# marbl/parsnp

Hardware: AMD Instinct MI355X
Metric: genomes/sec (MUM+LCB end-to-end) (higher is better)
Workload: dtype int32

## Files before the change

parsnp_amd/csrc/engine/engine_core.h:

```cpp
#pragma once
#include <algorithm>
#include <atomic>
#include <chrono>
#include <cstdint>
#include <cstdio>
#include <cstdlib>
#include <cstring>
#include <memory>
#include <mutex>
#include <new>
#include <string>
#include <thread>
#include <vector>

#include "kernels.h"
#include "store_kernels.h"
#include "dense_kernels.h"
#include "index_kernels.h"
#include "snp_kernels.h"
#include "nj_kernels.h"

namespace pm {

struct HostPool {
// ... 177 lines not shown
    static constexpr size_t kCtrLost = kCtrBase + 7;
    static constexpr size_t kCtrWords = kCtrBase + 8;
    static_assert(kCtrErr < kCtrGrouped && kCtrGrouped < kCtrWide && kCtrWide + kCtrWideWords <= kCtrOverflow && kCtrOverflow < kCtrLost && kCtrLost < kCtrWords,
                  "the words of the counter block are distinct and inside it");

private:
    struct CallHint { int64_t units = 0, ncand = 0, nok = 0; };
    struct StoreCounts { int64_t ms_count, rg_count, layout_rows, rg_pkey_init; };
    StoreCounts store_mark() const { return StoreCounts{ms_count, rg_count, layout_rows, rg_pkey_init}; }
    void store_rewind(const StoreCounts& m) { ms_count = m.ms_count; rg_count = m.rg_count; layout_rows = m.layout_rows; rg_pkey_init = m.rg_pkey_init; }
    void store_reset() { store_rewind(StoreCounts{0, 0, -1, 0}); }

    struct SearchCall {
        const int64_t nreg; const int64_t* const starts; const int64_t* const lens; const int32_t* const minsize; BatchResult* const out;
        const bool want_events, mumi; const GapBatch* const gb;
        bool from_store = false;
        int nq = 0, no_small = 0, lbits = 0;
        size_t nrow = 0, regz = 0, bytes_R = 0, bytes_pre = 0;
        int64_t npairs = 0, npos = 0, tsize = 0, fwords = 0, tsize_clear = 0, fwords_clear = 0, nbk = 0, npos_bucketed = 0, nchunks = 0, centries = 0, nwv = 0;
        RegionInfo* R = nullptr; int64_t *posbase = nullptr, *cbase = nullptr, *stage = nullptr;
        std::vector<int64_t> bbase;
        uint32_t* d_err = nullptr;
        int64_t nflag = 0; uint64_t ovf_cap = 0; bool index_counts_read = false;
        CallHint none; CallHint* hint = nullptr;
        int64_t nunits = 0; bool units_known = false;
        size_t ev_guess = 0, slice_cap = 0, queue_cap = 0, grp_cap = 0;
        uint64_t nev = 0, nrest = 0, ngrp = 0, worst_slice = 0;
        uint32_t errbits = 0, sticky = 0;
        bool first_form = false, wide_form = false, grouping = false, by_buckets = false, coarse_by_buckets = false, sharded = false;
        uint64_t *skey = nullptr, *sval = nullptr;
        const int64_t* ncand_p = nullptr; bool anchor_guess = false;
        bool exact = false, anchor_call = false;
        int64_t ncand_i = 0, nok = 0; uint64_t ncand = 0; size_t nokz = 0; const int64_t* nok_p = nullptr;
        std::vector<uint64_t> counts, qcounts; int64_t nunits_live = 0;
        int32_t verdict = 0;
        std::vector<int32_t> reg_h; int64_t counts_h[2] = {0, 0};
    };
    static constexpr int kNext = 1, kRepeat = 2;

    int run_once(int64_t nreg, const int64_t* starts, const int64_t* lens, const int32_t* minsize, BatchResult* out, bool want_events,
                 bool mumi, const GapBatch* gb = nullptr) {
        SearchCall c{nreg, starts, lens, minsize, out, want_events, mumi, gb};
        int rc = plan_call(c);
        if (rc != kNext) return rc;
        upload_and_clear(c);
        if ((rc = build_index(c)) != kNext) return rc;
        if ((rc = count_units(c)) != kNext) return rc;
        if ((rc = search_events(c)) != kNext) return rc;
        order_events(c);
        if (mumi) return mumi_tail(c);
        if ((rc = master_ep(c)) != kNext) return rc;
        return candidate_tail(c);
    }

    int plan_call(SearchCall& c) {
        const int64_t nreg = c.nreg; const int64_t* const starts = c.starts; const int64_t* const lens = c.lens; const int32_t* const minsize = c.minsize;
        BatchResult* const out = c.out; const GapBatch* const gb = c.gb;
        timing.clear();
        const int nq = c.nq = ngen - 1;
        out->nregions = nreg; out->nq = nq; out->total = 0;
        out->off.assign((size_t)nreg + 1, 0);
        out->release();
        out->pool = pool;
        if (nreg == 0) return 0;
        if (nq < 1) { error = "need at least one query genome"; return -2; }
        const int no_small = c.no_small = c.mumi ? 1 : 0;
// ... 511 lines not shown
            if (coll.allgather(coll.ctx, send.data(), (int64_t)(sizeof(GenomeAtK) * send.size()), recv.data())) { error = "all-gather of candidate states failed"; return -4; }
            for (int r = 0; r < coll.world; r++) {
                int a, b; shard_range(ngen, r, coll.world, &a, &b);
                const GenomeAtK* src = recv.data() + (size_t)r * send.size();
                for (size_t k = 0; k < cz; k++)
                    for (int x = 0; x < b - a; x++) all[k * nqz + (size_t)(a - 1 + x)] = src[k * (size_t)widest + (size_t)x];
            }
            be.h2d(d_at.p, all.data(), sizeof(GenomeAtK) * all.size());
        }
        be.mark("fold");
        return 0;
    }

    int tail_attempt(SearchCall& c, const bool exact) {
        const int64_t nreg = c.nreg, nwv = c.nwv; const int nq = c.nq, lbits = c.lbits; const GapBatch* const gb = c.gb; BatchResult* const out = c.out;
        const bool from_store = c.from_store, sharded = c.sharded; CallHint& hint = *c.hint;
        uint64_t* const skey = c.skey; uint64_t* const sval = c.sval; const int64_t* const ncand_p = c.ncand_p;
        const int32_t& verdict = c.verdict;
        int64_t &ncand_i = c.ncand_i, &nok = c.nok; int64_t (&counts_h)[2] = c.counts_h; std::vector<int32_t>& reg_h = c.reg_h;
        c.exact = exact;
        ncand_i = 0;
        if (exact) be.d2h(&ncand_i, ncand_p, 8);
        if (verdict < 0) { budget_exceeded = true; error = "per-thread work budget exceeded on some rank (degenerate repeat structure in a region)"; return -5; }
        if (exact) {
            last_candidates = ncand_i;
            if (ncand_i == 0) { hint.ncand = 1; hint.nok = 0; if (resident && from_store) out->store_base = ms_count; be.mark(nullptr); collect_timing(); return 0; }
        }
        const uint64_t ncand = c.ncand = exact ? (uint64_t)ncand_i : (uint64_t)(hint.ncand + hint.ncand / 8 + 256);
        ensure(d_cand, (size_t)ncand);
        be.launch("cand_write", nwv * 64, CandWrite{d_R.p, nreg, d_posbase.p, d_wmask.p, d_woff.p, d_cand.p, ncand});
        const uint64_t* scand = d_cand.p;

        be.mark("fold");
        ensure(d_ok, (size_t)ncand); ensure(d_ok_k, (size_t)ncand); ensure(d_ok_lon, (size_t)ncand);
        ensure(d_osp, (size_t)ncand * (size_t)nq); ensure(d_ofwd, (size_t)ncand * (size_t)nq);
        const GenomeAtK* at = nullptr;
        if (sharded) {
            if (int rc = exchange_states(c)) return rc;
            at = d_at.p;
        }
        be.launch_wave("fold_candidates", xcd_grid((int64_t)ncand),
                       FoldCandidates{d_R.p, scand, ngen, at, skey, sval, d_lo.p, d_state.p, d_rep.p, lbits, d_cbase.p, d_coarse.p,
                                      d_ok_k.p, d_ok_lon.p, d_osp.p, d_ofwd.p, d_ok.p, (int64_t)ncand, ncand_p});

        be.mark("compact");
        ensure(d_okcnt, (size_t)ncand + 1); ensure(d_okpos, (size_t)ncand + 1);
        be.launch("ok_count", (int64_t)ncand + 1, OkCount{d_ok.p, ncand_p, d_okcnt.p, (int64_t)ncand});
        be.exclusive_scan(d_okcnt.p, d_okpos.p, (size_t)ncand + 1);
        const int64_t* nok_p = c.nok_p = d_okpos.p + ncand;
        nok = 0;
        if (exact) be.d2h(&nok, nok_p, 8);
        const size_t nokz = c.nokz = exact ? (size_t)nok : (size_t)ncand;
        ensure(d_creg, std::max<size_t>(nokz, 1)); ensure(d_ck, std::max<size_t>(nokz, 1)); ensure(d_clon, std::max<size_t>(nokz, 1));
        reg_h.assign(nokz, 0);
        out->release();
        out->kb = pool->take(4 * nokz); out->lonb = pool->take(4 * nokz);
        out->rows = want_rows; out->dirty_known = false; out->table_id = 0; out->store_base = -1;
        const StoreCounts before = store_mark();
        c.anchor_call = false;
        if (!want_rows) compact_sp(c); else compact_rows(c);
        be.d2h_async(reg_h.data(), d_creg.p, 4 * nokz);
        be.d2h_async(out->kb.p, d_ck.p, 4 * nokz);
        counts_h[0] = ncand_i; counts_h[1] = nok;
        if (!exact) { be.d2h_async(&counts_h[0], ncand_p, 8); be.d2h_async(&counts_h[1], nok_p, 8); }
        flush_downloads();
        be.mark(nullptr);
        be.sync();
        const bool anchor_call = c.anchor_call;
        if (!exact) {
            ncand_i = counts_h[0]; nok = counts_h[1];
            const bool fits = (uint64_t)ncand_i <= ncand && anchor_call == (nreg == 1 && !gb && nok >= dirty_min);
            if (!fits) {
                store_rewind(before);
                tail_repeats++;
                be.mark("candidates");
                return kRepeat;
            }
            last_candidates = ncand_i;
            if (out->store_base >= 0) ms_count = out->store_base + nok;
        }
        hint.ncand = std::max<int64_t>(ncand_i, 1); hint.nok = nok;
        last_accepted = nok;
        if (anchor_call) { anchor_table_rows = nok; anchor_table_id = out->table_id; }
        for (int64_t w = 0; w < nok; w++) out->off[(size_t)reg_h[(size_t)w] + 1]++;
        for (int64_t r = 0; r < nreg; r++) out->off[(size_t)r + 1] += out->off[(size_t)r];
        out->total = out->off[(size_t)nreg];
        if (out->table_id && out->store_base == 0) anchor_flags_h.assign(out->flags(), out->flags() + nok);
        return kNext;
    }

    void compact_sp(SearchCall& c) {
        const int nq = c.nq; const uint64_t ncand = c.ncand; const size_t nokz = c.nokz, nqz2 = (size_t)nq; BatchResult* const out = c.out;
        const uint64_t* const scand = d_cand.p; const int64_t* const ncand_p = c.ncand_p;
        ensure(d_csp, std::max<size_t>(nokz * nqz2, 1)); ensure(d_cfwd, std::max<size_t>(nokz * nqz2, 1));
        be.launch("compact_sp", (int64_t)ncand * nq,
                  CompactSp{scand, d_ok.p, d_okpos.p, nq, d_ok_k.p, d_ok_lon.p, d_osp.p, d_ofwd.p, d_creg.p, d_ck.p, d_clon.p, d_csp.p, d_cfwd.p, ncand_p});
        be.mark("download");
        group_downloads();
        out->spb = pool->take(4 * nokz * nqz2); out->fwdb = pool->take(nokz * nqz2);
        be.d2h_async(out->spb.p, d_csp.p, 4 * nokz * nqz2);
        be.d2h_async(out->fwdb.p, d_cfwd.p, nokz * nqz2);
        be.d2h_async(out->lonb.p, d_clon.p, 4 * nokz);
    }

    void compact_rows(SearchCall& c) {
        const int64_t nreg = c.nreg; const GapBatch* const gb = c.gb; const bool from_store = c.from_store, exact = c.exact, anchor_guess = c.anchor_guess;
        const int64_t nok = c.nok; const uint64_t ncand = c.ncand; const size_t nokz = c.nokz, ngz = (size_t)ngen; BatchResult* const out = c.out;
        const uint64_t* const scand = d_cand.p; const int64_t* const ncand_p = c.ncand_p; const int64_t* const nok_p = c.nok_p;
        bool& anchor_call = c.anchor_call;
        anchor_call = nreg == 1 && !gb && (exact ? nok >= dirty_min : anchor_guess);
        const bool keep_rows = resident && (anchor_call || from_store);
        const bool to_store = anchor_call || keep_rows;
        int32_t* p_start; uint8_t* p_strand; int32_t* p_lon; uint32_t* p_flags;
        if (to_store) {
            if (anchor_call) store_reset();
            const size_t base = (size_t)ms_count, upto = base + nokz;
            ensure_keep(d_anchor_start, std::max<size_t>(upto * ngz, 1), base * ngz); ensure_keep(d_ms_strand, std::max<size_t>(upto * ngz, 1), base * ngz);
            ensure_keep(d_anchor_lon, std::max<size_t>(upto, 1), base); ensure_keep(d_anchor_flags, std::max<size_t>(upto, 1), base);
            ensure_keep(d_ms_shift, std::max<size_t>(upto, 1), base); ensure_keep(d_ms_len, std::max<size_t>(upto, 1), base); ensure_keep(d_ms_state, std::max<size_t>(upto, 1), base);
            p_start = d_anchor_start.p + base * ngz; p_strand = d_ms_strand.p + base * ngz; p_lon = d_anchor_lon.p + base; p_flags = d_anchor_flags.p + base;
            out->store_base = (int64_t)base;
            ms_count = (int64_t)upto;
        } else {
            ensure(d_csp, std::max<size_t>(nokz * ngz, 1)); ensure(d_cfwd, std::max<size_t>(nokz * ngz, 1)); ensure(d_cflags, std::max<size_t>(nokz, 1));
            p_start = d_csp.p; p_strand = d_cfwd.p; p_lon = d_clon.p; p_flags = d_cflags.p;
        }
        const bool long_list = nreg == 1 && (exact ? nok >= dirty_min : anchor_guess);
        if (long_list) ensure(d_dirty, nokz);
        {
            const ClearJob jobs[] = {{p_flags, 4 * nokz, 0}, {long_list ? d_dirty.p : nullptr, long_list ? 4 * nokz : 0, 0},
                                     {to_store ? d_ms_shift.p + (ms_count - (int64_t)nokz) : nullptr, to_store ? 4 * nokz : 0, 0},
                                     {to_store ? d_ms_state.p + (ms_count - (int64_t)nokz) : nullptr, to_store ? nokz : 0, 0}};
            be.clear_many(jobs, 4);
        }
        be.launch("compact_candidates", (int64_t)ncand * ngen,
                  CompactCandidates{scand, d_ok.p, d_okpos.p, ngen, d_ok_k.p, d_ok_lon.p, d_osp.p, d_ofwd.p, d_starts.p, d_lens.p, d_glen,
                                    d_creg.p, d_ck.p, p_lon, p_start, p_strand, p_flags, ncand_p});
        if (long_list) {
            const int64_t nblocks = ((int64_t)nokz + kDirtyBlock - 1) / kDirtyBlock, groups = (ngen + 63) / 64;
            ensure(d_bmax, (size_t)nblocks * ngz); ensure(d_bmin, (size_t)nblocks * ngz);
            be.launch_wave("dirty_extent", nblocks * groups, DirtyExtent{p_start, p_lon, p_flags, nok_p, ngen, d_bmax.p, d_bmin.p});
            be.launch_wave("dirty_prefix", groups, DirtyPrefix{nblocks, ngen, d_bmax.p, d_bmin.p});
            be.launch_wave("dirty_mark", nblocks * groups, DirtyMark{p_start, p_lon, nok_p, ngen, d_bmax.p, d_bmin.p, p_flags, d_dirty.p});
            be.launch("dirty_merge", (int64_t)nokz, DirtyMerge{d_dirty.p, p_flags, nok_p});
            out->dirty_known = true;
        }
        if (to_store) {
            be.d2d(d_ms_len.p + (ms_count - (int64_t)nokz), p_lon, 4 * nokz);
            if (anchor_call) out->table_id = ++table_counter;
        }
        be.mark("download");
        group_downloads();
        out->flagsb = pool->take(4 * nokz);
        be.d2h_async(out->flagsb.p, p_flags, 4 * nokz);
        if (!keep_rows) {
            out->startb = pool->take(4 * nokz * ngz); out->strandb = pool->take(nokz * ngz);
            be.d2h_async(out->startb.p, p_start, 4 * nokz * ngz);
            be.d2h_async(out->strandb.p, p_strand, nokz * ngz);
        }
        be.d2h_async(out->lonb.p, p_lon, 4 * nokz);
    }

public:

    bool resident = false;
    int64_t ms_count = 0;
    int64_t rg_count = 0;
    std::vector<RegInfo> rg_info_h;
    std::vector<uint32_t> anchor_flags_h;
    static constexpr int kAgain = -6;

    void reset_call_counts() {
        last_positions = last_candidates = last_accepted = last_grouped = last_grouped_wide = last_wide_regions = 0; last_handed_back = -1;
        last_index_bucketed = last_index_overflow = 0; last_index_lost = -1; last_alg[0] = last_alg[1] = last_alg[2] = 0;
    }
    void begin_store_call() { timing.clear(); last_events = last_rest = 0; reset_call_counts(); }
    Store store_view() { return Store{d_anchor_start.p, d_ms_strand.p, d_anchor_lon.p, d_anchor_flags.p, d_ms_shift.p, d_ms_len.p, d_ms_state.p, ngen}; }
    Layout layout_view(uint64_t* image, bool coherent = true) { return Layout{image, d_lay_off.p, d_lay_bits.p, coherent ? 1 : 0}; }
    size_t layout_geometry() {
        const size_t ngz = (size_t)ngen;
        if (lay_words == 0) {
// ... 785 lines not shown
            be.launch("dense_rerank", n, DenseRerank{d_dval2.p, d_dhead.p, d_dfirst.p, d_drank[k + 1].p});
            L.lv[k + 1] = d_drank[k + 1].p;
            be.d2h(&groups, d_dfirst.p + n, 8);
            if (groups == n) break;
        }
        if (groups != n) { error = "suffix-array sort did not converge"; return -5; }
        dense_rounds = k + 1;
        L.top = k;
        be.launch("dense_lcp", n, DenseLcp{L, d_dval2.p, d_dstart.p, nflag, d_dlcp.p});
        be.launch("dense_rep", n, DenseRep{d_R.p, d_dlist.p, d_dval2.p, d_dstart.p, nflag, d_dlcp.p, d_rep.p});
        return 0;
    }
    bool dense_mode = false;
    std::vector<uint8_t> dense_h;
    void collect_timing_more() { for (const PhaseTime& t : be.collect()) timing.push_back(t); }

    int allgather_host(const void* send, int64_t bytes, void* recv) {
        if (!coll.device) return coll.allgather(coll.ctx, send, bytes, recv);
        ensure(d_hsend, (size_t)bytes); ensure(d_hrecv, (size_t)bytes * (size_t)coll.world);
        be.h2d(d_hsend.p, send, (size_t)bytes);
        if (be.allgather_dev(d_hsend.p, bytes, d_hrecv.p)) return 1;
        be.d2h(recv, d_hrecv.p, (size_t)bytes * (size_t)coll.world);
        return 0;
    }

    std::vector<uint64_t> ev_key_h, ev_val_h;
    std::vector<int32_t> rep_h;
    int ev_lbits = 0;
    int64_t work_budget = 1 << 22;
    int64_t dirty_min = 4096;
    int64_t flagged_div = 8;
    int64_t tangled_max = 1 << 17;
    bool fast_tail = true;
    int64_t tail_repeats = 0;
    bool tangle_rounds = true;
    bool group_small = true;
    bool group_wide = false;
    int64_t last_grouped = 0;
    int64_t last_grouped_wide = 0, last_handed_back = -1, last_wide_regions = 0;
    bool force_atomic_marks = false;
    int filter_factor = 8;
    int slot_factor = 2;
    bool bucket_sort = true;
    bool index_build = true;
    int64_t index_bucket_min = 1 << 24;
    bool index_verify = false;
    int64_t index_overflow_cap = 0;
    int64_t last_index_bucketed = 0, last_index_overflow = 0, last_index_lost = -1;
    bool master_seg = true;
    bool force_gate = false;
    int64_t chain_window = 4096;
    int64_t chain_passed[2] = {-1, -1};
    bool force_chain_tie = false;
    bool force_unsure = false;
    bool order_debug = false;
    int64_t outside_writes = 0;
    int64_t exact_cluster_tests = 0;
    int64_t deferred_regions = 0;
    bool clusters_out_of_order = false;
    int64_t hint_shrink = 1;
    bool phase_timing = true;
    bool tune(const std::string& key, int64_t value) {
        if (key == "flagged_div" && value >= 1) { flagged_div = value; return true; }
        if (key == "tangled_max" && value >= 0) { tangled_max = value; return true; }
        if (key == "tangle_rounds") { tangle_rounds = value != 0; return true; }
        if (key == "fast_tail") { fast_tail = value != 0; return true; }
        if (key == "atomic_marks") { force_atomic_marks = value != 0; return true; }
        if (key == "master_seg") { master_seg = value != 0; return true; }
        if (key == "bucket_sort") { bucket_sort = value != 0; return true; }
        if (key == "index_build") { index_build = value != 0; return true; }
        if (key == "index_bucket_min" && value >= 1) { index_bucket_min = value; return true; }
        if (key == "index_verify") { index_verify = value != 0; return true; }
        if (key == "index_overflow_cap" && value >= 0) { index_overflow_cap = value; return true; }
        if (key == "filter_factor") { filter_factor = value < 1 ? 1 : (int)value; return true; }
        if (key == "slot_factor") { slot_factor = value < 1 ? 1 : (int)value; return true; }
        if (key == "stage_gate") { force_gate = value != 0; return true; }
        if (key == "chain_window" && value >= 1 && value <= kChainWindowMax) { chain_window = value; return true; }
        if (key == "chain_tie") { force_chain_tie = value != 0; return true; }
        if (key == "cluster_unsure") { force_unsure = value != 0; return true; }
        if (key == "order_debug") { order_debug = value != 0; return true; }
        if (key == "timing") { phase_timing = value != 0; be.timing_on = phase_timing; return true; }
        if (key == "group_small") { group_small = value != 0; return true; }
        if (key == "group_wide") { group_wide = value != 0; return true; }
        if (key == "work_budget" && value > 0) { work_budget = value; return true; }
        if (key == "dense_all") { dense_all = value != 0; return true; }
        if (key == "dirty_min" && value >= 0) { dirty_min = value; return true; }
        if (key == "hint_shrink" && value >= 1) { hint_shrink = value; return true; }
        if (key == "copy_kernel") { return tune_copy_kernel(be, value != 0, 0); }
        return false;
    }

    void release() {
        if (chain_event) { be.event_wait(chain_event); be.event_release(chain_event); chain_event = nullptr; }
        for (BufBase* b : all_bufs) { if (b->raw) be.free(b->raw); b->raw = nullptr; b->cap = 0; }
        if (chain_host) be.pinned_free(chain_host);
        chain_host = nullptr; chain_host_cap = 0; chain_pending = false;
        if (blk) be.free(blk);
        if (d_goff) be.free(d_goff);
        if (d_glen) be.free(d_glen);
// ... 23 lines not shown
        if (n <= b.cap && b.p) return;
        if (std::find(all_bufs.begin(), all_bufs.end(), (BufBase*)&b) == all_bufs.end()) all_bufs.push_back(&b);
        const size_t want = n + n / 2 + 16;
        void* raw = be.alloc(want * sizeof(T));
        if (!raw) throw DeviceOutOfMemory{want * sizeof(T)};
        if (b.p && keep) { be.d2d(raw, b.p, keep * sizeof(T)); be.sync(); }
        if (b.raw) be.free(b.raw);
        b.raw = raw; b.p = (T*)raw; b.cap = want;
    }
    void collect_timing() { timing = be.collect(); }
    template <class T> static auto group_on(T& b, int) -> decltype(b.d2h_group(), void()) { b.d2h_group(); }
    template <class T> static void group_on(T&, long) {}
    template <class T> static auto flush_on(T& b, int) -> decltype(b.d2h_flush(), void()) { b.d2h_flush(); }
    template <class T> static void flush_on(T&, long) {}
    template <class T> static auto tune_copy_kernel(T& b, bool on, int) -> decltype(b.group_copies = on, true) { b.group_copies = on; return true; }
    template <class T> static bool tune_copy_kernel(T&, bool, long) { return true; }
    template <class T> static auto sort_keys_on(T& b, uint64_t* ki, uint64_t* ko, size_t n, int lo, int hi, int) -> decltype(b.sort_keys(ki, ko, n, lo, hi), true) { b.sort_keys(ki, ko, n, lo, hi); return true; }
    template <class T> static bool sort_keys_on(T&, uint64_t*, uint64_t*, size_t, int, int, long) { return false; }
    void group_downloads() { group_on(be, 0); }
    void flush_downloads() { flush_on(be, 0); }

    SeqBlock* blk = nullptr; int64_t* d_goff = nullptr; int64_t* d_glen = nullptr;
    Packed P{};
    size_t ev_cap_hint = 0, rest_cap_hint[2] = {0, 0}, grp_cap_hint = 0;
    std::vector<CallHint> call_hints;
    int64_t call_ordinal = 0;
    Buf<uint8_t> d_gflag; Buf<int64_t> d_glo;
    Buf<int64_t> d_bkbase, d_bkbegin, d_ovf; Buf<uint64_t> d_ikey, d_ikey2, d_ikey3, d_ikey4;
    Buf<RegionInfo> d_R; Buf<int64_t> d_starts, d_lens, d_posbase;
    Buf<uint64_t> d_slots; Buf<uint32_t> d_filter, d_repeated; Buf<int32_t> d_next, d_rep, d_run, d_epm;
    Buf<int64_t> d_ucount, d_uoff; Buf<UnitRec> d_units;
    Buf<uint64_t> d_counter, d_evkey, d_evval, d_evkey2, d_evval2, d_evkey3, d_evval3; Buf<int64_t> d_sliceoff;
    Buf<int64_t> d_lo, d_cov; Buf<EventAtK> d_state; Buf<PairState> d_wsummary, d_wcarry; Buf<int32_t> d_emax;
    Buf<uint64_t> d_cand; Buf<GenomeAtK> d_at; Buf<uint8_t> d_ok; Buf<int32_t> d_ok_k, d_ok_lon, d_osp; Buf<uint8_t> d_ofwd;
    Buf<uint64_t> d_wmask; Buf<int64_t> d_wcount, d_woff;
    Buf<int64_t> d_bcount, d_bbegin, d_pbase;
    Buf<int64_t> d_okcnt, d_okpos, d_cbase; Buf<int32_t> d_coarse; Buf<int32_t> d_creg, d_ck, d_clon, d_csp; Buf<uint8_t> d_cfwd;
    Buf<uint32_t> d_cflags, d_dirty; Buf<int32_t> d_bmax, d_bmin;
    Buf<GenomeAtK> d_xsend, d_xrecv; Buf<uint8_t> d_hsend, d_hrecv;
    Buf<RestItem> d_rest; Buf<uint64_t> d_qcount;
    Buf<uint8_t> d_dense; Buf<int32_t> d_dfi, d_dlist, d_dlcp; Buf<int64_t> d_dstart, d_dhead, d_dfirst;
    Buf<uint64_t> d_dkey, d_dkey2, d_dval, d_dval2; Buf<uint32_t> d_drank[kDenseMaxLevels];
    Buf<int32_t> d_anchor_start, d_anchor_lon; Buf<uint32_t> d_anchor_flags;
    int64_t table_counter = 0;
    Buf<uint64_t> d_image;
    Buf<int64_t> d_un_blk, d_un_cnt, d_un_scan, d_un_tot; Buf<int32_t> d_un_out;
    Buf<double> d_nj_D, d_nj_R, d_nj_q; Buf<uint8_t> d_nj_active; Buf<int32_t> d_nj_j, d_nj_dist; Buf<NjJoinRec> d_nj_joins; Buf<NjLastRec> d_nj_last;
    Buf<uint64_t> d_snp_counts, d_snp_lo, d_snp_hi; Buf<uint8_t> d_snp_chunk; Buf<int64_t> d_snp_flag, d_snp_rank, d_snp_col; Buf<int32_t> d_snp_dist;
    Buf<uint8_t> d_ms_strand, d_ms_state, d_small8, d_o_strand; Buf<int32_t> d_ms_shift, d_ms_len, d_list, d_list2, d_j_min, d_j_max, d_o_start;
    Buf<int64_t> d_rg_start, d_rg_len, d_lay_off, d_lay_bits, d_v_row0, d_v_first, d_f_start, d_f_end, d_f_pack; Buf<RegInfo> d_rg_info; Buf<uint64_t> d_rg_count, d_once, d_twice;
    Buf<RowInfo> d_rowinfo; Buf<uint64_t> d_alg;
    Buf<int64_t> d_sd_cnt, d_sd_off; Buf<uint8_t> d_sd_keep;
    Buf<uint64_t> d_t_rem; Buf<uint8_t> d_t_done;
    Buf<int32_t> d_v_done, d_owner; Buf<uint8_t> d_v_defer, d_v_involved;
    Buf<uint64_t> d_t_left; uint64_t tangle_left[8] = {0, 0, 0, 0, 0, 0, 0, 0}; int tangle_ran = 0;
    Buf<int64_t> d_rg_pkey; Buf<OutsideWrite> d_outw; Buf<uint64_t> d_outw_count; int64_t rg_pkey_init = 0; uint64_t outside_writes_call = 0;
    Buf<ForeignRead> d_foreign; Buf<uint64_t> d_foreign_count, d_foreign_masks; Buf<int64_t> d_ms_key;
    size_t foreign_cap = 0; int64_t ms_key_rows = 0; uint64_t foreign_seen = 0;
    static constexpr size_t kHitCap = 256;
    Buf<uint64_t> d_hit_count, d_hit_owned, d_hit_present; Buf<int32_t> d_hits; Buf<uint8_t> d_recwords;
    Buf<int64_t> d_ch_flag, d_ch_pos, d_ch_head, d_ch_hpos, d_ch_survive, d_ch_spos, d_ch_hdr;
    Buf<uint64_t> d_ch_key, d_ch_val, d_ch_skey, d_ch_srow, d_ch_key2, d_ch_row2, d_ch_lcblen;
    Buf<uint8_t> d_ch_verdict, d_ch_outhead; Buf<int32_t> d_ch_outrow;
    Buf<int64_t> d_ch_back, d_ch_wflag, d_ch_wpos, d_ch_wlist, d_ch_wend; Buf<uint8_t> d_ch_wverdict, d_ch_wkeep;
    uint8_t* chain_host = nullptr; size_t chain_host_cap = 0; void* chain_event = nullptr; bool chain_pending = false; int64_t chain_cap = 0;
    size_t lay_words = 0, rg_cap_hint = 0;
    int64_t layout_rows = -1;
// ... 4 lines not shown
```

parsnp_amd/csrc/engine/kernels.h:

```cpp
#pragma once
#include <cstdint>

#if defined(__HIPCC__)
#define PM_HD __host__ __device__ inline
#else
#define PM_HD inline
#endif

namespace pm {

PM_HD int ctz64(uint64_t x) {
#if defined(__HIP_DEVICE_COMPILE__)
    return __ffsll((unsigned long long)x) - 1;
#else
    return __builtin_ctzll(x);
#endif
}
PM_HD int clz64(uint64_t x) {
#if defined(__HIP_DEVICE_COMPILE__)
    return __clzll((long long)x);
#else
    return __builtin_clzll(x);
#endif
}
// ... 1600 lines not shown
        if (tid < npos) { const RegionInfo& ri = R[upper_slot(posbase, nregions, tid)]; hit = cand_hit(ri, epm, (int32_t)(tid - ri.posbase)); }
        const unsigned long long m = __ballot(hit);
        if (__lane_id() == 0) { wmask[w] = m; wcount[w] = __popcll(m); }
#else
        uint64_t m = 0;
        for (int t = 0; t < 64 && w * 64 + t < npos; t++) {
            const int64_t tid = w * 64 + t;
            const RegionInfo& ri = R[upper_slot(posbase, nregions, tid)];
            if (cand_hit(ri, epm, (int32_t)(tid - ri.posbase))) m |= 1ull << t;
        }
        wmask[w] = m; wcount[w] = __builtin_popcountll(m);
#endif
    }
};
struct CandWrite {
    const RegionInfo* R; int64_t nregions; const int64_t* posbase; const uint64_t* wmask; const int64_t* woff;
    uint64_t* cand; uint64_t cand_cap;
    PM_HD void operator()(int64_t tid) const {
        const uint64_t m = wmask[tid >> 6];
        const int t = (int)(tid & 63);
        if (!((m >> t) & 1)) return;
        const uint64_t at = (uint64_t)woff[tid >> 6] + (uint64_t)
#if defined(__HIP_DEVICE_COMPILE__)
            __popcll(m & ((1ull << t) - 1));
#else
            __builtin_popcountll(m & ((1ull << t) - 1));
#endif
        if (at >= cand_cap) return;
        const int64_t r = upper_slot(posbase, nregions, tid);
        cand[at] = ((uint64_t)r << 32) | (uint32_t)(tid - R[r].posbase);
    }
};

struct GenomeAtK { int32_t epf, upf, spf, epr, upr, spr; };
PM_HD GenomeAtK state_at(const RegionInfo& ri, int64_t r, int32_t k, int g, int32_t nq, const uint64_t* key, const uint64_t* val,
                         const int64_t* lo, const EventAtK* st, const int32_t* rep, int lbits, const int64_t* cbase, const int32_t* coarse) {
    const int64_t pair = r * nq + g;
    const int32_t* row = coarse + cbase[r] * nq + (int64_t)(k >> kCoarseShift) * nq;
    const int64_t first = lo[pair];
    int64_t a = first + row[g], b = first + row[nq + g];
    const uint64_t want = ((((uint64_t)pair << lbits) | (uint64_t)k) << 1) | 1ull;
    while (a < b) { const int64_t mid = (a + b) >> 1; if (key[mid] <= want) a = mid + 1; else b = mid; }
    GenomeAtK o{0, 0, 0, 0, 0, 0};
    if (a > first) {
        const EventAtK s = st[a - 1];
        if (s.s[0].e1) { o.epf = s.s[0].e1; o.upf = s.s[0].up; o.spf = s.s[0].spb + k; }
        if (s.s[1].e1) { o.epr = s.s[1].e1; o.upr = s.s[1].up; o.spr = s.s[1].spb + k; }
    }
    return o;
}
struct StateAtCandidate {
    const RegionInfo* R; const uint64_t* cand; int32_t ngen; const uint64_t* key; const uint64_t* val; const int64_t* lo;
    const EventAtK* st; const int32_t* rep; int lbits; GenomeAtK* out;
    const int64_t* cbase; const int32_t* coarse;
    PM_HD void operator()(int64_t tid) const {
        const int32_t nq = ngen - 1;
        const int64_t c = tid / nq; const int g = (int)(tid % nq);
        const int64_t r = (int64_t)(cand[c] >> 32); const int32_t k = (int32_t)(cand[c] & 0xffffffffu);
        out[tid] = state_at(R[r], r, k, g, nq, key, val, lo, st, rep, lbits, cbase, coarse);
    }
};
struct PackStates {
    const GenomeAtK* at; int32_t nq; int32_t g0; int32_t mine; int32_t widest; GenomeAtK* send;
    PM_HD void operator()(int64_t tid) const {
        const int64_t c = tid / widest; const int x = (int)(tid % widest);
        send[tid] = x < mine ? at[c * nq + g0 + x] : GenomeAtK{0, 0, 0, 0, 0, 0};
    }
};
struct UnpackStates {
    const GenomeAtK* recv; int32_t nq; int32_t world; int32_t widest; int64_t ncand; GenomeAtK* at;
    PM_HD void operator()(int64_t tid) const {
        const int64_t c = tid / nq; const int g = (int)(tid % nq);
        int r = (int)(((int64_t)(g + 1) * world - 1) / nq);
        while (r > 0 && (int)((int64_t)nq * r / world) > g) r--;
        while (r + 1 < world && (int)((int64_t)nq * (r + 1) / world) <= g) r++;
        const int first = (int)((int64_t)nq * r / world);
        at[tid] = recv[(int64_t)r * ncand * widest + c * widest + (g - first)];
    }
};

struct FoldCandidates {
    const RegionInfo* R; const uint64_t* cand; int32_t ngen; const GenomeAtK* at;
    const uint64_t* key; const uint64_t* val; const int64_t* lo; const EventAtK* st; const int32_t* rep; int lbits;
    const int64_t* cbase; const int32_t* coarse;
    int32_t* out_k; int32_t* out_lon; int32_t* out_sp; uint8_t* out_fwd; uint8_t* out_ok;
    int64_t ncand;
    const int64_t* count;
    PM_HD void wave(int64_t w) const {
        const int64_t nc = *count < ncand ? *count : ncand;
        if (w / kXcds >= (nc + kXcds - 1) / kXcds) return;
        const int64_t c = xcd_item(w, nc);
        if (c >= nc) return;
        const int32_t nq = ngen - 1;
        const int64_t r = (int64_t)(cand[c] >> 32); const int32_t k = (int32_t)(cand[c] & 0xffffffffu);
        const RegionInfo& ri = R[r];
        int32_t em = ri.nR, um = 0;
#if defined(__HIP_DEVICE_COMPILE__)
        const int lane = (int)__lane_id();
        for (int g0 = 0; g0 < nq; g0 += 64) {
            const int g = g0 + lane;
            const bool act = g < nq;
            GenomeAtK s{0, 0, 0, 0, 0, 0};
            if (act) s = at ? at[c * nq + g] : state_at(ri, r, k, g, nq, key, val, lo, st, rep, lbits, cbase, coarse);
            const int32_t m = act ? (s.epf > s.epr ? s.epf : s.epr) : 0x7fffffff;
            const int32_t incl = wave_incl_min(m);
            int32_t before = __shfl_up(incl, 1, 64);
            if (lane == 0 || before > em) before = em;
            const int32_t fe = before < s.epf ? before : s.epf, re = before < s.epr ? before : s.epr;
            const bool fwd = fe > re;
            const int32_t u = act ? (fwd ? s.upf : s.upr) : 0;
            if (act) { out_sp[c * nq + g] = fwd ? s.spf : s.spr; out_fwd[c * nq + g] = fwd ? 1 : 0; }
            const int32_t last = __shfl(incl, 63, 64);
            if (last < em) em = last;
            const int32_t umax = wave_all_max(u);
            if (umax > um) um = umax;
        }
        if (lane == 0) { out_k[c] = k; out_lon[c] = em - k; out_ok[c] = (um < em && em - k >= ri.minsize) ? 1 : 0; }
#else
        for (int g = 0; g < nq; g++) {
            const GenomeAtK s = at ? at[c * nq + g] : state_at(ri, r, k, g, nq, key, val, lo, st, rep, lbits, cbase, coarse);
            const int32_t fe = em < s.epf ? em : s.epf, fu = um > s.upf ? um : s.upf;
            const int32_t re = em < s.epr ? em : s.epr, ru = um > s.upr ? um : s.upr;
            if (fe > re) { em = fe; um = fu; out_sp[c * nq + g] = s.spf; out_fwd[c * nq + g] = 1; }
            else { em = re; um = ru; out_sp[c * nq + g] = s.spr; out_fwd[c * nq + g] = 0; }
        }
        out_k[c] = k; out_lon[c] = em - k;
        out_ok[c] = (um < em && em - k >= ri.minsize) ? 1 : 0;
#endif
    }
};

struct OkCount {
    const uint8_t* ok; const int64_t* ncand; int64_t* cnt; int64_t cap;
    PM_HD void operator()(int64_t c) const { cnt[c] = (c < *ncand && c < cap) ? (ok[c] ? 1 : 0) : 0; }
};
struct CompactSp {
    const uint64_t* cand; const uint8_t* ok; const int64_t* pos; int32_t nq;
    const int32_t* k; const int32_t* lon; const int32_t* sp; const uint8_t* fwd;
    int32_t* out_region; int32_t* out_k; int32_t* out_lon; int32_t* out_sp; uint8_t* out_fwd;
    const int64_t* ncand;
    PM_HD void operator()(int64_t tid) const {
        const int64_t c = tid / nq; const int g = (int)(tid % nq);
        if (c >= *ncand || !ok[c]) return;
        const int64_t w = pos[c];
        out_sp[w * nq + g] = sp[tid]; out_fwd[w * nq + g] = fwd[tid];
        if (g == 0) { out_region[w] = (int32_t)(cand[c] >> 32); out_k[w] = k[c]; out_lon[w] = lon[c]; }
    }
};
constexpr uint32_t kRowBad = 1;
constexpr uint32_t kRowOutside = 2;
constexpr uint32_t kRowReverse = 4;
constexpr uint32_t kRowDirty = 8;
constexpr uint32_t kRowEarly = 16;
struct CompactCandidates {
    const uint64_t* cand; const uint8_t* ok; const int64_t* pos; int32_t ngen;
    const int32_t* k; const int32_t* lon; const int32_t* sp; const uint8_t* fwd;
    const int64_t* starts; const int64_t* lens; const int64_t* glen;
    int32_t* out_region; int32_t* out_k; int32_t* out_lon; int32_t* out_start; uint8_t* out_strand; uint32_t* out_flags;
    const int64_t* ncand;
    PM_HD void operator()(int64_t tid) const {
        const int64_t c = tid / ngen; const int j = (int)(tid % ngen);
        if (c >= *ncand || !ok[c]) return;
        const int64_t w = pos[c];
        const int64_t r = (int64_t)(cand[c] >> 32);
        const int64_t lo = lon[c];
        const int64_t ws = starts[r * ngen + j], wl = lens[r * ngen + j];
        int64_t st; uint32_t f, bits = 0;
        if (j == 0) {
            st = (int64_t)k[c] + ws; f = 1;
            if ((uint64_t)k[c] + 1 > (uint64_t)(uint32_t)wl) bits |= kRowBad;
            out_region[w] = (int32_t)r; out_k[w] = k[c]; out_lon[w] = lon[c];
        } else {
            const int64_t q = sp[c * (ngen - 1) + j - 1];
            f = fwd[c * (ngen - 1) + j - 1];
            if ((uint64_t)q + 1 > (uint64_t)(uint32_t)wl) bits |= kRowBad;
            const int64_t at = q + ws;
            st = f ? at : glen[j] - (at + lo);
            if (!f) bits |= kRowReverse;
        }
        if (st + lo > glen[j] || st < 0) bits |= kRowOutside;
        out_start[w * ngen + j] = (int32_t)st; out_strand[w * ngen + j] = (uint8_t)f;
        if (bits) atomic_or32(&out_flags[w], bits);
    }
};

constexpr int kDirtyBlock = 256;
// ... 111 lines not shown
```

Baseline: 31890.

## Fold candidate rows directly into final row layout and close holes in place

The fold kernel can now write per-genome start, strand and flags rows straight into the destination buffers (store or compact arrays), indexed by candidate. It no longer writes intermediate sp/fwd arrays that a separate compact_candidates kernel would then reformat. A two-pass shift kernel then moves accepted rows down to their compacted positions, and is skipped when all candidates are accepted. Because the anchor decision must be made before the fold, a wrong guess now forces a repeat of the tail; destination buffers are also sized by candidate count rather than accepted count.

```diff
diff --git a/parsnp_amd/csrc/engine/engine_core.h b/parsnp_amd/csrc/engine/engine_core.h
--- a/parsnp_amd/csrc/engine/engine_core.h
+++ b/parsnp_amd/csrc/engine/engine_core.h
@@ -233,6 +233,8 @@
         const int64_t* ncand_p = nullptr; bool anchor_guess = false;
         bool exact = false, anchor_call = false;
         int64_t ncand_i = 0, nok = 0; uint64_t ncand = 0; size_t nokz = 0; const int64_t* nok_p = nullptr;
+        int32_t* p_start = nullptr; uint8_t* p_strand = nullptr; int32_t* p_lon = nullptr; uint32_t* p_flags = nullptr; bool to_store = false, keep_rows = false;
+        int anchor_known = -1;
         std::vector<uint64_t> counts, qcounts; int64_t nunits_live = 0;
         int32_t verdict = 0;
         std::vector<int32_t> reg_h; int64_t counts_h[2] = {0, 0};
@@ -810,16 +812,34 @@
         const uint64_t* scand = d_cand.p;
 
         be.mark("fold");
+        const bool rows_fold = want_rows && fold_rows;
+        const size_t ocols = rows_fold ? (size_t)ngen : (size_t)nq;
         ensure(d_ok, (size_t)ncand); ensure(d_ok_k, (size_t)ncand); ensure(d_ok_lon, (size_t)ncand);
-        ensure(d_osp, (size_t)ncand * (size_t)nq); ensure(d_ofwd, (size_t)ncand * (size_t)nq);
+        ensure(d_osp, (size_t)ncand * ocols); ensure(d_ofwd, (size_t)ncand * ocols);
         const GenomeAtK* at = nullptr;
         if (sharded) {
             if (int rc = exchange_states(c)) return rc;
             at = d_at.p;
         }
-        be.launch_wave("fold_candidates", xcd_grid((int64_t)ncand),
-                       FoldCandidates{d_R.p, scand, ngen, at, skey, sval, d_lo.p, d_state.p, d_rep.p, lbits, d_cbase.p, d_coarse.p,
-                                      d_ok_k.p, d_ok_lon.p, d_osp.p, d_ofwd.p, d_ok.p, (int64_t)ncand, ncand_p});
+        out->release();
+        out->rows = want_rows; out->dirty_known = false; out->table_id = 0; out->store_base = -1;
+        const StoreCounts before = store_mark();
+        c.anchor_call = false;
+        if (rows_fold) {
+            const bool anchor = nreg == 1 && !gb && (c.anchor_known >= 0 ? c.anchor_known != 0 : exact ? ncand_i >= dirty_min : c.anchor_guess);
+            ensure(d_creg, std::max<size_t>((size_t)ncand, 1)); ensure(d_ck, std::max<size_t>((size_t)ncand, 1)); ensure(d_clon, std::max<size_t>((size_t)ncand, 1));
+            ensure(d_ok_flags, (size_t)ncand);
+            rows_destination(c, (size_t)ncand, anchor);
+            const size_t base = c.to_store ? (size_t)out->store_base : 0;
+            const FoldRowDest row{d_starts.p, d_lens.p, d_glen, d_creg.p, c.p_start, c.p_strand, c.p_flags,
+                                  c.to_store ? d_ms_len.p + base : nullptr, c.to_store ? d_ms_shift.p + base : nullptr, c.to_store ? d_ms_state.p + base : nullptr};
+            be.launch_wave("fold_candidates", xcd_grid((int64_t)ncand),
+                           FoldCandidateRows{d_R.p, scand, ngen, at, skey, sval, d_lo.p, d_state.p, d_rep.p, lbits, d_cbase.p, d_coarse.p,
+                                             d_ck.p, c.p_lon, nullptr, nullptr, d_ok.p, (int64_t)ncand, ncand_p, row});
+        } else
+            be.launch_wave("fold_candidates", xcd_grid((int64_t)ncand),
+                           FoldCandidates{d_R.p, scand, ngen, at, skey, sval, d_lo.p, d_state.p, d_rep.p, lbits, d_cbase.p, d_coarse.p,
+                                          d_ok_k.p, d_ok_lon.p, d_osp.p, d_ofwd.p, d_ok.p, (int64_t)ncand, ncand_p, FoldRowDest{}});
 
         be.mark("compact");
         ensure(d_okcnt, (size_t)ncand + 1); ensure(d_okpos, (size_t)ncand + 1);
@@ -828,16 +848,17 @@
         const int64_t* nok_p = c.nok_p = d_okpos.p + ncand;
         nok = 0;
         if (exact) be.d2h(&nok, nok_p, 8);
+        if (rows_fold && exact) {
+            const bool anchor = nreg == 1 && !gb && nok >= dirty_min;
+            if (anchor != c.anchor_call) { c.anchor_known = anchor ? 1 : 0; tail_again(c, before); return kRepeat; }
+            if (c.to_store) ms_count = out->store_base + nok;
+        }
         const size_t nokz = c.nokz = exact ? (size_t)nok : (size_t)ncand;
-        ensure(d_creg, std::max<size_t>(nokz, 1)); ensure(d_ck, std::max<size_t>(nokz, 1)); ensure(d_clon, std::max<size_t>(nokz, 1));
+        if (!rows_fold) { ensure(d_creg, std::max<size_t>(nokz, 1)); ensure(d_ck, std::max<size_t>(nokz, 1)); ensure(d_clon, std::max<size_t>(nokz, 1)); }
         reg_h.assign(nokz, 0);
-        out->release();
         out->kb = pool->take(4 * nokz); out->lonb = pool->take(4 * nokz);
-        out->rows = want_rows; out->dirty_known = false; out->table_id = 0; out->store_base = -1;
-        const StoreCounts before = store_mark();
-        c.anchor_call = false;
-        if (!want_rows) compact_sp(c); else compact_rows(c);
-        be.d2h_async(reg_h.data(), d_creg.p, 4 * nokz);
+        if (rows_fold) close_holes(c); else if (!want_rows) compact_sp(c); else compact_rows(c);
+        if (nokz) be.d2h_async(reg_h.data(), d_creg.p, 4 * nokz);
         be.d2h_async(out->kb.p, d_ck.p, 4 * nokz);
         counts_h[0] = ncand_i; counts_h[1] = nok;
         if (!exact) { be.d2h_async(&counts_h[0], ncand_p, 8); be.d2h_async(&counts_h[1], nok_p, 8); }
@@ -849,9 +870,8 @@
             ncand_i = counts_h[0]; nok = counts_h[1];
             const bool fits = (uint64_t)ncand_i <= ncand && anchor_call == (nreg == 1 && !gb && nok >= dirty_min);
             if (!fits) {
-                store_rewind(before);
-                tail_repeats++;
-                be.mark("candidates");
+                if ((uint64_t)ncand_i <= ncand) c.anchor_known = nreg == 1 && !gb && nok >= dirty_min ? 1 : 0;
+                tail_again(c, before);
                 return kRepeat;
             }
             last_candidates = ncand_i;
@@ -881,28 +901,57 @@
         be.d2h_async(out->lonb.p, d_clon.p, 4 * nokz);
     }
 
-    void compact_rows(SearchCall& c) {
-        const int64_t nreg = c.nreg; const GapBatch* const gb = c.gb; const bool from_store = c.from_store, exact = c.exact, anchor_guess = c.anchor_guess;
-        const int64_t nok = c.nok; const uint64_t ncand = c.ncand; const size_t nokz = c.nokz, ngz = (size_t)ngen; BatchResult* const out = c.out;
-        const uint64_t* const scand = d_cand.p; const int64_t* const ncand_p = c.ncand_p; const int64_t* const nok_p = c.nok_p;
-        bool& anchor_call = c.anchor_call;
-        anchor_call = nreg == 1 && !gb && (exact ? nok >= dirty_min : anchor_guess);
-        const bool keep_rows = resident && (anchor_call || from_store);
-        const bool to_store = anchor_call || keep_rows;
-        int32_t* p_start; uint8_t* p_strand; int32_t* p_lon; uint32_t* p_flags;
-        if (to_store) {
-            if (anchor_call) store_reset();
-            const size_t base = (size_t)ms_count, upto = base + nokz;
+    void rows_destination(SearchCall& c, const size_t rows, const bool anchor) {
+        const size_t ngz = (size_t)ngen; BatchResult* const out = c.out;
+        c.anchor_call = anchor;
+        c.keep_rows = resident && (anchor || c.from_store);
+        c.to_store = anchor || c.keep_rows;
+        if (c.to_store) {
+            if (anchor) store_reset();
+            const size_t base = (size_t)ms_count, upto = base + rows;
             ensure_keep(d_anchor_start, std::max<size_t>(upto * ngz, 1), base * ngz); ensure_keep(d_ms_strand, std::max<size_t>(upto * ngz, 1), base * ngz);
             ensure_keep(d_anchor_lon, std::max<size_t>(upto, 1), base); ensure_keep(d_anchor_flags, std::max<size_t>(upto, 1), base);
             ensure_keep(d_ms_shift, std::max<size_t>(upto, 1), base); ensure_keep(d_ms_len, std::max<size_t>(upto, 1), base); ensure_keep(d_ms_state, std::max<size_t>(upto, 1), base);
-            p_start = d_anchor_start.p + base * ngz; p_strand = d_ms_strand.p + base * ngz; p_lon = d_anchor_lon.p + base; p_flags = d_anchor_flags.p + base;
+            c.p_start = d_anchor_start.p + base * ngz; c.p_strand = d_ms_strand.p + base * ngz; c.p_lon = d_anchor_lon.p + base; c.p_flags = d_anchor_flags.p + base;
             out->store_base = (int64_t)base;
             ms_count = (int64_t)upto;
         } else {
-            ensure(d_csp, std::max<size_t>(nokz * ngz, 1)); ensure(d_cfwd, std::max<size_t>(nokz * ngz, 1)); ensure(d_cflags, std::max<size_t>(nokz, 1));
-            p_start = d_csp.p; p_strand = d_cfwd.p; p_lon = d_clon.p; p_flags = d_cflags.p;
-        }
+            ensure(d_csp, std::max<size_t>(rows * ngz, 1)); ensure(d_cfwd, std::max<size_t>(rows * ngz, 1)); ensure(d_cflags, std::max<size_t>(rows, 1));
+            c.p_start = d_csp.p; c.p_strand = d_cfwd.p; c.p_lon = d_clon.p; c.p_flags = d_cflags.p;
+        }
+    }
+
+    void tail_again(SearchCall& c, const StoreCounts& before) {
+        if (c.anchor_call && before.ms_count > 0) anchor_table_id = 0;
+        store_rewind(before);
+        tail_repeats++;
+        be.mark("candidates");
+    }
+
+    void close_holes(SearchCall& c) {
+        const uint64_t ncand = c.ncand;
+        const FoldRowsShift shift{d_cand.p, d_ok.p, d_okpos.p, c.ncand_p, c.nok_p, (int64_t)ncand, ngen, d_creg.p, d_ck.p, c.p_lon, c.p_start, c.p_strand, c.p_flags,
+                                  c.to_store ? d_ms_len.p + c.out->store_base : nullptr, d_ok_k.p, d_ok_lon.p, d_osp.p, d_ofwd.p, d_ok_flags.p, 0,
+                                  std::min<int64_t>((int64_t)ncand, 4096)};
+        FoldRowsShift back = shift; back.back = 1;
+        be.launch_wave("fold_rows_out", shift.nwaves, shift);
+        be.launch_wave("fold_rows_back", back.nwaves, back);
+        const bool long_list = c.nreg == 1 && (c.exact ? c.nok >= dirty_min : c.anchor_guess);
+        if (long_list) {
+            ensure(d_dirty, c.nokz);
+            const ClearJob job{d_dirty.p, 4 * c.nokz, 0};
+            be.clear_many(&job, 1);
+        }
+        rows_tail(c, long_list);
+    }
+
+    void compact_rows(SearchCall& c) {
+        const int64_t nreg = c.nreg; const GapBatch* const gb = c.gb; const bool exact = c.exact, anchor_guess = c.anchor_guess;
+        const int64_t nok = c.nok; const uint64_t ncand = c.ncand; const size_t nokz = c.nokz;
+        const uint64_t* const scand = d_cand.p; const int64_t* const ncand_p = c.ncand_p;
+        rows_destination(c, nokz, nreg == 1 && !gb && (exact ? nok >= dirty_min : anchor_guess));
+        const bool to_store = c.to_store;
+        int32_t* const p_start = c.p_start; uint8_t* const p_strand = c.p_strand; int32_t* const p_lon = c.p_lon; uint32_t* const p_flags = c.p_flags;
         const bool long_list = nreg == 1 && (exact ? nok >= dirty_min : anchor_guess);
         if (long_list) ensure(d_dirty, nokz);
         {
@@ -914,6 +963,13 @@
         be.launch("compact_candidates", (int64_t)ncand * ngen,
                   CompactCandidates{scand, d_ok.p, d_okpos.p, ngen, d_ok_k.p, d_ok_lon.p, d_osp.p, d_ofwd.p, d_starts.p, d_lens.p, d_glen,
                                     d_creg.p, d_ck.p, p_lon, p_start, p_strand, p_flags, ncand_p});
+        rows_tail(c, long_list);
+    }
+
+    void rows_tail(SearchCall& c, const bool long_list) {
+        const size_t nokz = c.nokz, ngz = (size_t)ngen; BatchResult* const out = c.out; const int64_t* const nok_p = c.nok_p;
+        const bool to_store = c.to_store, keep_rows = c.keep_rows, anchor_call = c.anchor_call;
+        int32_t* const p_start = c.p_start; uint8_t* const p_strand = c.p_strand; int32_t* const p_lon = c.p_lon; uint32_t* const p_flags = c.p_flags;
         if (long_list) {
             const int64_t nblocks = ((int64_t)nokz + kDirtyBlock - 1) / kDirtyBlock, groups = (ngen + 63) / 64;
             ensure(d_bmax, (size_t)nblocks * ngz); ensure(d_bmin, (size_t)nblocks * ngz);
@@ -924,7 +980,7 @@
             out->dirty_known = true;
         }
         if (to_store) {
-            be.d2d(d_ms_len.p + (ms_count - (int64_t)nokz), p_lon, 4 * nokz);
+            if (!fold_rows) be.d2d(d_ms_len.p + (ms_count - (int64_t)nokz), p_lon, 4 * nokz);
             if (anchor_call) out->table_id = ++table_counter;
         }
         be.mark("download");
@@ -1776,6 +1832,7 @@
     int64_t flagged_div = 8;
     int64_t tangled_max = 1 << 17;
     bool fast_tail = true;
+    bool fold_rows = true;
     int64_t tail_repeats = 0;
     bool tangle_rounds = true;
     bool group_small = true;
@@ -1809,6 +1866,7 @@
         if (key == "tangled_max" && value >= 0) { tangled_max = value; return true; }
         if (key == "tangle_rounds") { tangle_rounds = value != 0; return true; }
         if (key == "fast_tail") { fast_tail = value != 0; return true; }
+        if (key == "fold_rows") { fold_rows = value != 0; return true; }
         if (key == "atomic_marks") { force_atomic_marks = value != 0; return true; }
         if (key == "master_seg") { master_seg = value != 0; return true; }
         if (key == "bucket_sort") { bucket_sort = value != 0; return true; }
@@ -1898,7 +1956,7 @@
     Buf<int64_t> d_ucount, d_uoff; Buf<UnitRec> d_units;
     Buf<uint64_t> d_counter, d_evkey, d_evval, d_evkey2, d_evval2, d_evkey3, d_evval3; Buf<int64_t> d_sliceoff;
     Buf<int64_t> d_lo, d_cov; Buf<EventAtK> d_state; Buf<PairState> d_wsummary, d_wcarry; Buf<int32_t> d_emax;
-    Buf<uint64_t> d_cand; Buf<GenomeAtK> d_at; Buf<uint8_t> d_ok; Buf<int32_t> d_ok_k, d_ok_lon, d_osp; Buf<uint8_t> d_ofwd;
+    Buf<uint64_t> d_cand; Buf<GenomeAtK> d_at; Buf<uint8_t> d_ok; Buf<int32_t> d_ok_k, d_ok_lon, d_osp; Buf<uint8_t> d_ofwd; Buf<uint32_t> d_ok_flags;
     Buf<uint64_t> d_wmask; Buf<int64_t> d_wcount, d_woff;
     Buf<int64_t> d_bcount, d_bbegin, d_pbase;
     Buf<int64_t> d_okcnt, d_okpos, d_cbase; Buf<int32_t> d_coarse; Buf<int32_t> d_creg, d_ck, d_clon, d_csp; Buf<uint8_t> d_cfwd;
diff --git a/parsnp_amd/csrc/engine/kernels.h b/parsnp_amd/csrc/engine/kernels.h
--- a/parsnp_amd/csrc/engine/kernels.h
+++ b/parsnp_amd/csrc/engine/kernels.h
@@ -1656,6 +1656,11 @@
     }
 };
 
+constexpr uint32_t kRowBad = 1;
+constexpr uint32_t kRowOutside = 2;
+constexpr uint32_t kRowReverse = 4;
+constexpr uint32_t kRowDirty = 8;
+constexpr uint32_t kRowEarly = 16;
 struct GenomeAtK { int32_t epf, upf, spf, epr, upr, spr; };
 PM_HD GenomeAtK state_at(const RegionInfo& ri, int64_t r, int32_t k, int g, int32_t nq, const uint64_t* key, const uint64_t* val,
                          const int64_t* lo, const EventAtK* st, const int32_t* rep, int lbits, const int64_t* cbase, const int32_t* coarse) {
@@ -1703,13 +1708,36 @@
     }
 };
 
-struct FoldCandidates {
+struct FoldRowDest {
+    const int64_t* starts; const int64_t* lens; const int64_t* glen;
+    int32_t* region; int32_t* start; uint8_t* strand; uint32_t* flags;
+    int32_t* ms_len; int32_t* ms_shift; uint8_t* ms_state;
+};
+template <bool kRows>
+struct FoldCandidatesT {
     const RegionInfo* R; const uint64_t* cand; int32_t ngen; const GenomeAtK* at;
     const uint64_t* key; const uint64_t* val; const int64_t* lo; const EventAtK* st; const int32_t* rep; int lbits;
     const int64_t* cbase; const int32_t* coarse;
     int32_t* out_k; int32_t* out_lon; int32_t* out_sp; uint8_t* out_fwd; uint8_t* out_ok;
     int64_t ncand;
     const int64_t* count;
+    FoldRowDest row;
+    PM_HD uint32_t put(int64_t c, int64_t r, int j, int64_t q, bool fwd, int64_t& over, bool& neg) const {
+        const int64_t ws = row.starts[r * ngen + j], wl = row.lens[r * ngen + j];
+        const int64_t a = q + ws, d = a - row.glen[j];
+        if (d > over) over = d;
+        if (a < 0) neg = true;
+        row.start[c * ngen + j] = (int32_t)a; row.strand[c * ngen + j] = fwd ? 1 : 0;
+        return ((uint64_t)q + 1 > (uint64_t)(uint32_t)wl ? kRowBad : 0u) | (fwd ? 0u : kRowReverse);
+    }
+    PM_HD void flip(int64_t c, int j, int64_t lon) const {
+        int32_t* const p = &row.start[c * ngen + j];
+        *p = (int32_t)(row.glen[j] - ((int64_t)*p + lon));
+    }
+    PM_HD void finish(int64_t c, int64_t r, int32_t k, int32_t lon, uint32_t bits) const {
+        row.region[c] = (int32_t)r; row.flags[c] = bits;
+        if (row.ms_len) { row.ms_len[c] = lon; row.ms_shift[c] = 0; row.ms_state[c] = 0; }
+    }
     PM_HD void wave(int64_t w) const {
         const int64_t nc = *count < ncand ? *count : ncand;
         if (w / kXcds >= (nc + kXcds - 1) / kXcds) return;
@@ -1719,6 +1747,8 @@
         const int64_t r = (int64_t)(cand[c] >> 32); const int32_t k = (int32_t)(cand[c] & 0xffffffffu);
         const RegionInfo& ri = R[r];
         int32_t em = ri.nR, um = 0;
+        int64_t over = -(int64_t(1) << 62); bool neg = false;
+        uint32_t bits = 0, rev = 0;
 #if defined(__HIP_DEVICE_COMPILE__)
         const int lane = (int)__lane_id();
         for (int g0 = 0; g0 < nq; g0 += 64) {
@@ -1733,24 +1763,78 @@
             const int32_t fe = before < s.epf ? before : s.epf, re = before < s.epr ? before : s.epr;
             const bool fwd = fe > re;
             const int32_t u = act ? (fwd ? s.upf : s.upr) : 0;
-            if (act) { out_sp[c * nq + g] = fwd ? s.spf : s.spr; out_fwd[c * nq + g] = fwd ? 1 : 0; }
+            if constexpr (kRows) {
+                if (act) {
+                    bits |= put(c, r, g + 1, fwd ? s.spf : s.spr, fwd, over, neg);
+                    if (!fwd) rev |= 1u << (g0 >> 6);
+                }
+            } else if (act) { out_sp[c * nq + g] = fwd ? s.spf : s.spr; out_fwd[c * nq + g] = fwd ? 1 : 0; }
             const int32_t last = __shfl(incl, 63, 64);
             if (last < em) em = last;
             const int32_t umax = wave_all_max(u);
             if (umax > um) um = umax;
         }
+        if constexpr (kRows) {
+            const int64_t lon = em - k;
+            for (uint32_t m = rev; m; m &= m - 1) flip(c, 64 * (__ffs((int)m) - 1) + lane + 1, lon);
+            if (lane == 0) bits |= put(c, r, 0, k, true, over, neg);
+            if (neg || over + lon > 0) bits |= kRowOutside;
+            bits = wave_all_or(bits);
+            if (lane == 0) finish(c, r, k, em - k, bits);
+        }
         if (lane == 0) { out_k[c] = k; out_lon[c] = em - k; out_ok[c] = (um < em && em - k >= ri.minsize) ? 1 : 0; }
 #else
         for (int g = 0; g < nq; g++) {
             const GenomeAtK s = at ? at[c * nq + g] : state_at(ri, r, k, g, nq, key, val, lo, st, rep, lbits, cbase, coarse);
             const int32_t fe = em < s.epf ? em : s.epf, fu = um > s.upf ? um : s.upf;
             const int32_t re = em < s.epr ? em : s.epr, ru = um > s.upr ? um : s.upr;
-            if (fe > re) { em = fe; um = fu; out_sp[c * nq + g] = s.spf; out_fwd[c * nq + g] = 1; }
-            else { em = re; um = ru; out_sp[c * nq + g] = s.spr; out_fwd[c * nq + g] = 0; }
+            const bool fwd = fe > re;
+            if (fwd) { em = fe; um = fu; } else { em = re; um = ru; }
+            if constexpr (kRows) bits |= put(c, r, g + 1, fwd ? s.spf : s.spr, fwd, over, neg);
+            else { out_sp[c * nq + g] = fwd ? s.spf : s.spr; out_fwd[c * nq + g] = fwd ? 1 : 0; }
+        }
+        if constexpr (kRows) {
+            (void)rev;
+            for (int j = 1; j < ngen; j++) if (!row.strand[c * ngen + j]) flip(c, j, em - k);
+            bits |= put(c, r, 0, k, true, over, neg);
+            if (neg || over + (em - k) > 0) bits |= kRowOutside;
+            finish(c, r, k, em - k, bits);
         }
         out_k[c] = k; out_lon[c] = em - k;
         out_ok[c] = (um < em && em - k >= ri.minsize) ? 1 : 0;
 #endif
+    }
+};
+using FoldCandidates = FoldCandidatesT<false>;
+using FoldCandidateRows = FoldCandidatesT<true>;
+
+struct FoldRowsShift {
+    const uint64_t* cand; const uint8_t* ok; const int64_t* pos; const int64_t* ncand; const int64_t* nok; int64_t cap; int32_t ngen;
+    int32_t* region; int32_t* k; int32_t* lon; int32_t* start; uint8_t* strand; uint32_t* flags; int32_t* ms_len;
+    int32_t* t_k; int32_t* t_lon; int32_t* t_start; uint8_t* t_strand; uint32_t* t_flags;
+    int back; int64_t nwaves;
+    PM_HD void wave(int64_t w0) const {
+        const int64_t nc = *ncand < cap ? *ncand : cap;
+        if (*nok == nc) return;
+        for (int64_t c = w0; c < nc; c += nwaves) if (ok[c] && pos[c] != c) move(c);
+    }
+    PM_HD void move(int64_t c) const {
+        const int64_t w = pos[c];
+#if defined(__HIP_DEVICE_COMPILE__)
+        const int j0 = (int)__lane_id(), dj = 64;
+#else
+        const int j0 = 0, dj = 1;
+#endif
+        if (!back) {
+            for (int j = j0; j < ngen; j += dj) { t_start[c * ngen + j] = start[c * ngen + j]; t_strand[c * ngen + j] = strand[c * ngen + j]; }
+            if (j0 == 0) { t_k[c] = k[c]; t_lon[c] = lon[c]; t_flags[c] = flags[c]; }
+        } else {
+            for (int j = j0; j < ngen; j += dj) { start[w * ngen + j] = t_start[c * ngen + j]; strand[w * ngen + j] = t_strand[c * ngen + j]; }
+            if (j0 == 0) {
+                region[w] = (int32_t)(cand[c] >> 32); k[w] = t_k[c]; lon[w] = t_lon[c]; flags[w] = t_flags[c];
+                if (ms_len) ms_len[w] = t_lon[c];
+            }
+        }
     }
 };
 
@@ -1771,11 +1855,6 @@
         if (g == 0) { out_region[w] = (int32_t)(cand[c] >> 32); out_k[w] = k[c]; out_lon[w] = lon[c]; }
     }
 };
-constexpr uint32_t kRowBad = 1;
-constexpr uint32_t kRowOutside = 2;
-constexpr uint32_t kRowReverse = 4;
-constexpr uint32_t kRowDirty = 8;
-constexpr uint32_t kRowEarly = 16;
 struct CompactCandidates {
     const uint64_t* cand; const uint8_t* ok; const int64_t* pos; int32_t ngen;
     const int32_t* k; const int32_t* lon; const int32_t* sp; const uint8_t* fwd;
```

Result: no change. 32190, median of 6 (+0.9%).
